# risingwavelabs/risingwave

Measured on AMD Instinct MI355X. Metric: input rows/sec/GPU on Nexmark q7 stream, higher is better.
Workload: dtype int64; 1 GPU; nexmark_q7; chunk_rows=4096, chunks_per_epoch_step=4096, windows_per_epoch=64, barriers=one checkpoint flush per step (a step = one epoch), agg=max(price), count group by 10s window (append-only), parallelism=dp1

## Files before the change

### include/rw_stream.h

```cpp
#ifndef RW_STREAM_H
#define RW_STREAM_H

#include "rw_chunk.h"

#ifdef __cplusplus
extern "C" {
#endif

#define RW_OK 0
#define RW_E_INVAL (-1)
#define RW_E_OVERFLOW (-2)
#define RW_E_INCONSISTENT (-3)
#define RW_E_NOGPU (-4)
#define RW_E_INTERNAL (-5)

const char* rw_last_error(void);
void rw_chunk_free(RwChunk* c);


enum RwAggKind {
    RW_AGG_COUNT_STAR = 0,
    RW_AGG_COUNT = 1,
    RW_AGG_SUM = 2,
    RW_AGG_SUM0 = 3,
// ... 94 lines not shown

void* rw_hash_join_create(const RwHashJoinDesc* desc);
int rw_hash_join_push_chunk(void* h, int side, const RwChunk* chunk);
int rw_hash_join_flush(void* h, uint64_t epoch);
int rw_hash_join_ingest_mode(void* h, int epoch_batched);
RwChunk* rw_hash_join_poll(void* h);
void rw_hash_join_destroy(void* h);

int rw_hash_join_watermark(void* h, int side, uint32_t col_idx, int64_t val,
                           uint32_t* out_cols, int64_t* out_vals, int max_out);

int rw_hash_agg_watermark(void* h, uint32_t group_key_pos, int64_t val);

int rw_hash_agg_update_vnode_bitmap(void* h, const uint8_t* bitmap,
                                    uint32_t vnode_count);
int rw_hash_join_update_vnode_bitmap(void* h, const uint8_t* bitmap,
                                     uint32_t vnode_count);

typedef struct RwGroupTopNDesc {
    uint32_t n_cols;
    const uint8_t* types;
    uint32_t n_group_by;
    const uint32_t* group_by;
    uint32_t n_order_by;
    const uint32_t* order_cols;
    const uint8_t* order_desc;
    uint32_t n_rest;
    const uint32_t* rest_cols;
    const uint8_t* rest_desc;
    uint64_t offset;
    uint64_t limit;
    uint8_t with_ties;
    uint32_t chunk_size;
    uint64_t state_capacity_hint;
    uint64_t row_capacity_hint;
} RwGroupTopNDesc;

void* rw_group_top_n_create(const RwGroupTopNDesc* desc);
int rw_group_top_n_push_chunk(void* h, const RwChunk* chunk);
int rw_group_top_n_flush(void* h, uint64_t epoch);
RwChunk* rw_group_top_n_poll(void* h);
void rw_group_top_n_destroy(void* h);

int rw_agg_checkpoint_drain(void* h, uint8_t** buf, uint64_t* len);
int rw_hash_agg_restore(void* h, const uint8_t* buf, uint64_t len);
int rw_agg_n_minput_tables(void* h);
int rw_agg_minput_drain(void* h, int mi, uint8_t** buf, uint64_t* len);
int rw_agg_minput_restore(void* h, int mi, const uint8_t* buf, uint64_t len);
int rw_hash_join_restore(void* h, int side, const uint8_t* buf, uint64_t len,
                         const uint8_t* deg_buf, uint64_t deg_len);
int rw_join_checkpoint_drain(void* h, int side, uint8_t** buf, uint64_t* len);
int rw_join_compact(void* h, int side, uint64_t* reclaimed);

int rw_hash_join_varlen_reserve(void* h, int side, uint64_t bytes);
int rw_hash_join_varlen_stats(void* h, int side, uint64_t* used,
                              uint64_t* capacity);
int rw_hash_join_varlen_emit_stats(void* h, double* ms, double* copy_ms,
                                   uint64_t* bytes, uint64_t* launches);
int rw_hash_agg_varlen_reserve(void* h, uint64_t arena_bytes,
                               uint64_t n_strings);
int rw_hash_agg_varlen_stats(void* h, uint64_t* arena_used,
                             uint64_t* arena_cap, uint64_t* n_strings,
                             uint64_t* table_cap);
int rw_hash_agg_varlen_intern_stats(void* h, double* kernel_ms,
                                    double* fetch_ms, uint64_t* launches);
int rw_agg_minput_compact(void* h, uint64_t* reclaimed);
int rw_topn_compact(void* h, uint64_t* reclaimed);
int rw_topn_checkpoint_drain(void* h, uint8_t** buf, uint64_t* len);
int rw_topn_restore(void* h, const uint8_t* buf, uint64_t len);
int rw_group_top_n_watermark(void* h, uint32_t col_idx, int64_t val);
int rw_agg_n_dedup_tables(void* h);
int rw_agg_dedup_drain(void* h, int di, uint8_t** buf, uint64_t* len);
int rw_agg_dedup_restore(void* h, int di, const uint8_t* buf, uint64_t len);
int rw_join_degree_drain(void* h, int side, uint8_t** buf, uint64_t* len);
void rw_spill_free(uint8_t* buf);

int rw_agg_apply_flush_launch(void* h, void* batch, uint32_t r0, uint32_t r1,
                              uint64_t epoch);
int rw_agg_debug_set_fuse(void* h, int mode);
int rw_agg_debug_fuse_allowed(void* h);
long long rw_agg_debug_fused_launches(void* h);
uint32_t rw_agg_debug_fuse_max(void);

#ifdef __cplusplus
}
#endif
#endif
```

### risingwave_amd/csrc/rw_amd.hip

```cpp

#include <hip/hip_runtime.h>

#include <cstdint>
#include <cstdio>
#include <cstdlib>
#include <cstring>
#include <map>
#include <new>
#include <optional>
#include <string>
#include <unordered_set>
#include <vector>

#include <rocprim/device/device_scan.hpp>

#include "../../include/rw_codec.hpp"
#include "../../include/rw_stream.h"
#include "../../include/rw_varlen.hpp"
#include "../../include/rw_xpayload.hpp"

#define WAVE 64

static thread_local std::string g_err;

// ... 5421 lines not shown
            }
        } else if (active && mhead != UINT32_MAX) {
            uint32_t row = mhead;
            while (row != UINT32_MAX) {
                JoinRowHdr* h = jrow(match, row);
                uint32_t vb = ld_u32(&h->validbits);
                if (ld_u32(&h->alive) &&
                    jhdr_key_eq(h, m.key_cols[1 - S], m.KW, kw, nullmask,
                                true) &&
                    join_cond_ok(m, S, b, r, vb, jvals(h))) {
                    const long long* mv = jvals(h);
                    jemit_row(out, m, S, op, b, r, vb,
                              [&](int col) {
                                  return ld_i64((const int64_t*)&mv[col]);
                              },
                              3);
                    matched_row = row;
                }
                row = ld_u32(&h->next);
            }
        }

        if (!m.append_only) {
            if (r < r1) {
                uint32_t myrow = *row_base + r;
                bool do_insert = active && is_insert;
                if (myrow < own.row_cap) {
                    JoinRowHdr* hd2 = jrow(own, myrow);
                    if (do_insert) {
                        long long* hv2 = jvals(hd2);
                        uint32_t vb2 = 0;
                        if (dense) {
                            for (int c = 0; c < m.n_cols[S]; c++)
                                hv2[c] = b.col_vals[c][r];
                            vb2 = (1u << m.n_cols[S]) - 1;
                            hd2->validbits = vb2;
                            hd2->degree = 0;
                            hd2->alive = 1;
                        } else if (b.all_insert) {
                            for (int c = 0; c < m.n_cols[S]; c++) {
                                hv2[c] = b.col_vals[c][r];
                                vb2 |= (uint32_t)(b.col_valid[c][r] != 0) << c;
                            }
                            hd2->validbits = vb2;
                            hd2->degree = 0;
                            hd2->alive = 1;
                        } else {
                            for (int c = 0; c < m.n_cols[S]; c++) {
                                st_i64((int64_t*)&hv2[c], b.col_vals[c][r]);
                                vb2 |= (uint32_t)(b.col_valid[c][r] != 0) << c;
                            }
                            st_u32(&hd2->validbits, vb2);
                            st_u32(&hd2->degree, 0);
                            st_u32(&hd2->alive, 1);
                        }
                        jbucket_insert(own, h64, myrow, !b.all_insert);
                    } else {
                        hd2->alive = 0;
                    }
                }
                if (active && !is_insert)
                    jown_delete(own, m, S, b, r, kw, nullmask);
            }
            continue;
        }
        if (!active) continue;

        if (m.append_only && is_insert && matched_row != UINT32_MAX) {
            st_u32(&jrow(match, matched_row)->alive, 0);
            if (match.killed) {
                uint32_t kidx = atomicAdd(match.killed_cursor, 1u);
                if (kidx < match.killed_cap) match.killed[kidx] = matched_row;
            }
            continue;
        }

        if (is_insert)
            jown_insert(own, m, S, b, r, kw, nullmask, out, 0);
        else
            jown_delete(own, m, S, b, r, kw, nullmask);
    }
}

__global__ void join_restore_kernel(JoinBatchDev b, JoinSideDev sd,
                                    JoinMeta m, int S,
                                    const uint32_t* degrees, uint32_t* err) {
    uint32_t stride = gridDim.x * blockDim.x;
    int lane = threadIdx.x & 63;
    uint32_t n = b.n_rows;
    uint32_t iters = (n + stride - 1) / stride;
    for (uint32_t it = 0; it < iters; it++) {
        uint32_t r = it * stride + blockIdx.x * blockDim.x + threadIdx.x;
        bool active = r < n;
        uint64_t wmask = __ballot(active);
        if (!active) continue;
        int leader = 63 - __clzll(wmask);
        uint32_t base = 0;
        if (lane == leader)
            base = atomicAdd(sd.row_cursor, (uint32_t)__popcll(wmask));
        base = (uint32_t)__shfl((int)base, leader);
        uint32_t row = base + (uint32_t)__popcll(wmask & ((1ULL << lane) - 1));
        if (row >= sd.row_cap) {
            atomicExch(err, 3u);
            continue;
        }
        JoinRowHdr* hd = jrow(sd, row);
        long long* hv = jvals(hd);
        uint32_t vb = 0;
        for (int c = 0; c < m.n_cols[S]; c++) {
            hv[c] = b.col_vals[c][r];
            vb |= (uint32_t)(b.col_valid[c][r] != 0) << c;
        }
        hd->validbits = vb;
        hd->degree = degrees ? degrees[r] : 0;
        hd->alive = 1;
        int64_t kw[MAX_KW];
        uint32_t nm = 0;
        for (int i = 0; i < m.KW; i++) {
            uint8_t col = m.key_cols[S][i];
            bool valid = (vb >> col) & 1;
            kw[i] = valid ? hv[col] : 0;
            nm |= (uint32_t)(!valid) << i;
        }
        jbucket_insert(sd, hash_key(kw, nm, m.KW), row, false);
    }
}

__global__ void jgather_rows_kernel(JoinSideDev sd, const uint32_t* ids,
                                    uint32_t n, uint8_t* out) {
    uint32_t stride = gridDim.x * blockDim.x;
    for (uint32_t i = blockIdx.x * blockDim.x + threadIdx.x; i < n;
         i += stride) {
        const uint8_t* src = sd.rows + (size_t)ids[i] * sd.row_stride;
        uint8_t* dst = out + (size_t)i * sd.row_stride;
        for (uint32_t w = 0; w < sd.row_stride; w += 8)
            *(long long*)(dst + w) = *(const long long*)(src + w);
    }
}

__global__ void jcompact_copy_kernel(JoinSideDev oldsd, uint8_t* nrows,
                                     uint32_t* ncursor, uint32_t old_n) {
    uint32_t stride = gridDim.x * blockDim.x;
    int lane = threadIdx.x & 63;
    uint32_t iters = (old_n + stride - 1) / stride;
    for (uint32_t it = 0; it < iters; it++) {
        uint32_t r = it * stride + blockIdx.x * blockDim.x + threadIdx.x;
        bool alive = r < old_n && jrow(oldsd, r)->alive;
        uint64_t wmask = __ballot(alive);
        if (!alive) continue;
        int leader = 63 - __clzll(wmask);
        uint32_t base = 0;
        if (lane == leader)
            base = atomicAdd(ncursor, (uint32_t)__popcll(wmask));
        base = (uint32_t)__shfl((int)base, leader);
        uint32_t nr = base + (uint32_t)__popcll(wmask & ((1ULL << lane) - 1));
        const uint8_t* src = oldsd.rows + (size_t)r * oldsd.row_stride;
        uint8_t* dst = nrows + (size_t)nr * oldsd.row_stride;
        for (uint32_t wq = 0; wq < oldsd.row_stride; wq += 8)
            *(long long*)(dst + wq) = *(const long long*)(src + wq);
        ((JoinRowHdr*)dst)->next = UINT32_MAX;
    }
}

__global__ void jcompact_link_kernel(JoinSideDev sd, JoinMeta m, int S,
                                     uint32_t n) {
    uint32_t stride = gridDim.x * blockDim.x;
// ... 609 lines not shown
    HIP_TRY(rocprim::exclusive_scan(d_scan_tmp, tmp, d_vlens, d_voffs,
                                    (uint64_t)0, (size_t)n + 1,
                                    rocprim::plus<uint64_t>(), stream));
    uint64_t total = 0;
    HIP_TRY(hipMemcpyAsync(&total, d_voffs + n, 8, hipMemcpyDeviceToHost,
                           stream));
    HIP_TRY(hipStreamSynchronize(stream));
    if (total) {
        uint64_t padded = total + VARLEN_COPY_PAD;
        if (d_vbytes_cap < padded) {
            if (d_vbytes) hipFree(d_vbytes);
            d_vbytes = nullptr;
            d_vbytes_cap = 0;
            uint64_t cap = 1ull << 16;
            while (cap < padded) cap <<= 1;
            HIP_TRY(hipMalloc(&d_vbytes, cap));
            d_vbytes_cap = cap;
        }
        if (timed) HIP_TRY(hipEventRecord(vev2, stream));
        varlen_copy_launch(v, arena, d_voffs, n, total, d_vbytes, stream);
    }
    if (timed) {
        HIP_TRY(hipEventRecord(vev1, stream));
        HIP_TRY(hipEventSynchronize(vev1));
        float ms = 0;
        HIP_TRY(hipEventElapsedTime(&ms, vev0, vev1));
        vemit_ms += ms;
        if (total) {
            HIP_TRY(hipEventElapsedTime(&ms, vev2, vev1));
            vcopy_ms += ms;
        }
        vemit_bytes += total;
        vemit_launches++;
    }
    HIP_TRY(hipMemcpy(offs.data(), d_voffs, ((size_t)n + 1) * 8,
                      hipMemcpyDeviceToHost));
    bytes.resize(total);
    if (total)
        HIP_TRY(hipMemcpy(bytes.data(), d_vbytes, total,
                          hipMemcpyDeviceToHost));
    return RW_OK;
}

VarlenFetch::~VarlenFetch() {
    if (d_vlens) hipFree(d_vlens);
    if (d_voffs) hipFree(d_voffs);
    if (d_vbytes) hipFree(d_vbytes);
    if (d_scan_tmp) hipFree(d_scan_tmp);
    if (vev0) {
        hipEventDestroy(vev0);
        hipEventDestroy(vev1);
        if (vev2) hipEventDestroy(vev2);
    }
}

struct HashJoin {
    RwHashJoinDesc desc;
    JoinMeta m{};
    JoinSideDev side[2]{};
    JoinOutDev out{};
    hipStream_t stream;
    std::vector<uint8_t> out_types;
    std::vector<uint8_t> types[2];
    JoinBatchDev stage[2]{};
    uint32_t stage_cap[2] = {0, 0};
    std::vector<RwChunk*> outq;
    uint8_t* zeros = nullptr;
    uint8_t* d_vnode_bitmap = nullptr;
    uint16_t* d_vnode_hop = nullptr;
    uint32_t d_vnode_hop_cap = 0;
    struct Wm { bool has = false; int64_t val = 0; };
    std::vector<uint32_t> wm_pos;
    std::vector<uint8_t> wm_clean;
    std::vector<Wm> wm_side0, wm_side1, wm_out;
    std::vector<uint32_t> ineq_col[2];
    std::vector<uint8_t> ineq_larger, ineq_do_clean;
    std::vector<Wm> ineq_wm[2], ineq_out;
    static constexpr int EV_RING = 256;
    hipEvent_t ev0[EV_RING] = {}, ev1[EV_RING] = {};
    uint8_t ev_pending[EV_RING] = {};
    uint64_t ev_head = 0;
    double probe_ms_total = 0;
    uint64_t probe_launches = 0, probe_rows = 0;

    int ev_harvest(int slot) {
        if (!ev_pending[slot]) return RW_OK;
        HIP_TRY(hipEventSynchronize(ev1[slot]));
        float ms = 0;
        HIP_TRY(hipEventElapsedTime(&ms, ev0[slot], ev1[slot]));
        probe_ms_total += ms;
        ev_pending[slot] = 0;
        return RW_OK;
    }
    int ev_harvest_all() {
        for (int s = 0; s < EV_RING; s++)
            if (ev_harvest(s) != RW_OK) return RW_E_INTERNAL;
        return RW_OK;
    }

    int init(const RwHashJoinDesc* d) {
        if (!gpu_ok()) FAIL(RW_E_NOGPU, "risingwave_amd: no GPU visible (product path has no CPU fallback)");
        desc = *d;
        if (d->join_type > RW_JOIN_RIGHT_ANTI)
            FAIL(RW_E_INVAL, "unknown join type %d", d->join_type);
        if (d->append_only && d->join_type != RW_JOIN_INNER)
            FAIL(RW_E_INVAL, "append-only optimize kernel is inner-only this round");
        if (d->n_key < 1 || d->n_key > MAX_KW) FAIL(RW_E_INVAL, "n_key %u", d->n_key);
        if (d->n_cols_l > MAX_COLS || d->n_cols_r > MAX_COLS)
            FAIL(RW_E_INVAL, "too many columns for round-1 kernels");
        if (d->n_output > MAX_OUT) FAIL(RW_E_INVAL, "too many output columns");
        m.KW = (int)d->n_key;
        m.n_cols[0] = (int)d->n_cols_l;
        m.n_cols[1] = (int)d->n_cols_r;
        m.n_pk[0] = (int)d->n_pk_l;
        m.n_pk[1] = (int)d->n_pk_r;
        types[0].assign(d->types_l, d->types_l + d->n_cols_l);
        types[1].assign(d->types_r, d->types_r + d->n_cols_r);
        for (int s = 0; s < 2; s++)
            for (size_t c = 0; c < types[s].size(); c++) {
                uint8_t t = types[s][c];
                if (t == RW_T_VARCHAR)
                    m.vc_mask[s] |= (uint8_t)(1u << c);
                else if (t != RW_T_I64 && t != RW_T_TS)
                    FAIL(RW_E_INVAL, "column type %d unsupported on GPU "
                                     "(i64/ts, varchar payload only)", t);
            }
        {
            const char* sn[2] = {"left", "right"};
            auto is_vc = [&](int s, uint32_t col) {
                return col < types[s].size() && types[s][col] == RW_T_VARCHAR;
            };
            auto is_vc_cat = [&](uint32_t idx) {
                return idx < d->n_cols_l ? is_vc(0, idx)
                                         : is_vc(1, idx - d->n_cols_l);
            };
            for (uint32_t i = 0; i < d->n_key; i++) {
                if (is_vc(0, d->key_l[i]))
                    FAIL(RW_E_INVAL, "varchar %s column %u cannot be a join key",
                         sn[0], d->key_l[i]);
                if (is_vc(1, d->key_r[i]))
                    FAIL(RW_E_INVAL, "varchar %s column %u cannot be a join key",
                         sn[1], d->key_r[i]);
            }
            for (uint32_t i = 0; i < d->n_pk_l; i++)
                if (is_vc(0, d->pk_l[i]))
                    FAIL(RW_E_INVAL, "varchar %s column %u cannot be a pk column",
                         sn[0], d->pk_l[i]);
            for (uint32_t i = 0; i < d->n_pk_r; i++)
                if (is_vc(1, d->pk_r[i]))
                    FAIL(RW_E_INVAL, "varchar %s column %u cannot be a pk column",
                         sn[1], d->pk_r[i]);
            if (d->has_cond && (is_vc_cat(d->cond_l) || is_vc_cat(d->cond_r)))
                FAIL(RW_E_INVAL, "varchar column %u cannot be a condition operand",
                     is_vc_cat(d->cond_l) ? d->cond_l : d->cond_r);
            if (d->has_cond && d->has_cond2 &&
                (is_vc_cat(d->cond2_l) || is_vc_cat(d->cond2_r)))
                FAIL(RW_E_INVAL, "varchar column %u cannot be a condition operand",
                     is_vc_cat(d->cond2_l) ? d->cond2_l : d->cond2_r);
            for (uint32_t p = 0; p < d->n_ineq; p++) {
                if (is_vc(0, d->ineq_left_col[p]))
                    FAIL(RW_E_INVAL, "varchar %s column %u cannot be an "
                                     "inequality/watermark column",
                         sn[0], d->ineq_left_col[p]);
                if (is_vc(1, d->ineq_right_col[p]))
                    FAIL(RW_E_INVAL, "varchar %s column %u cannot be an "
                                     "inequality/watermark column",
                         sn[1], d->ineq_right_col[p]);
            }
        }
        for (uint32_t i = 0; i < d->n_key; i++) {
            m.key_cols[0][i] = (uint8_t)d->key_l[i];
            m.key_cols[1][i] = (uint8_t)d->key_r[i];
            if (d->null_safe[i]) m.null_safe_mask |= 1 << i;
        }
        if (d->n_pk_l > MAX_KW || d->n_pk_r > MAX_KW) FAIL(RW_E_INVAL, "pk too wide");
        for (uint32_t i = 0; i < d->n_pk_l; i++) m.pk_cols[0][i] = (uint8_t)d->pk_l[i];
        for (uint32_t i = 0; i < d->n_pk_r; i++) m.pk_cols[1][i] = (uint8_t)d->pk_r[i];
        m.n_out = (int)d->n_output;
        for (uint32_t i = 0; i < d->n_output; i++) {
            uint32_t idx = d->output_indices[i];
            if (idx < d->n_cols_l) {
                m.out_src[i] = 0;
                m.out_col[i] = (uint8_t)idx;
                out_types.push_back(types[0][idx]);
            } else {
                m.out_src[i] = 1;
                m.out_col[i] = (uint8_t)(idx - d->n_cols_l);
                out_types.push_back(types[1][idx - d->n_cols_l]);
            }
        }
        auto split = [&](uint32_t idx, uint8_t* src, uint8_t* col) {
            if (idx < d->n_cols_l) {
                *src = 0;
                *col = (uint8_t)idx;
            } else {
                *src = 1;
                *col = (uint8_t)(idx - d->n_cols_l);
            }
        };
        m.n_cond = 0;
        if (d->has_cond) {
            m.cond[0].op = d->cond_op;
            split(d->cond_l, &m.cond[0].src_l, &m.cond[0].col_l);
            split(d->cond_r, &m.cond[0].src_r, &m.cond[0].col_r);
            m.cond[0].rconst = d->cond_rconst;
            m.n_cond = 1;
            if (d->has_cond2) {
                m.cond[1].op = d->cond2_op;
                split(d->cond2_l, &m.cond[1].src_l, &m.cond[1].col_l);
                split(d->cond2_r, &m.cond[1].src_r, &m.cond[1].col_r);
                m.cond[1].rconst = d->cond2_rconst;
                m.n_cond = 2;
            }
        }
        m.append_only = d->append_only;
        m.join_type = d->join_type;
        m.need_deg[0] = j_need_degree(d->join_type, RW_SIDE_LEFT);
        m.need_deg[1] = j_need_degree(d->join_type, RW_SIDE_RIGHT);
        if (d->n_wm_jk) {
            wm_pos.assign(d->wm_jk_pos, d->wm_jk_pos + d->n_wm_jk);
            wm_clean.assign(d->wm_jk_clean, d->wm_jk_clean + d->n_wm_jk);
        }
        wm_side0.resize(d->n_key);
        wm_side1.resize(d->n_key);
        wm_out.resize(d->n_key);
        if (d->n_ineq) {
            ineq_col[0].assign(d->ineq_left_col,
                               d->ineq_left_col + d->n_ineq);
            ineq_col[1].assign(d->ineq_right_col,
                               d->ineq_right_col + d->n_ineq);
            ineq_larger.assign(d->ineq_left_larger,
                               d->ineq_left_larger + d->n_ineq);
            ineq_do_clean.assign(d->ineq_clean, d->ineq_clean + d->n_ineq);
            ineq_wm[0].resize(d->n_ineq);
            ineq_wm[1].resize(d->n_ineq);
            ineq_out.resize(d->n_ineq);
        }

        HIP_TRY(hipStreamCreate(&stream));
        uint64_t key_cap = d->state_capacity_hint ? d->state_capacity_hint : (1u << 20);
        uint64_t row_cap = d->row_capacity_hint ? d->row_capacity_hint : (1u << 22);
        for (int s = 0; s < 2; s++) {
            uint32_t cap = 1;
            while (cap < key_cap * 2) cap <<= 1;
            JoinSideDev& js = side[s];
            js.cap_mask = cap - 1;
            js.slots = nullptr;
            HIP_TRY(hipMalloc(&js.slots8, (size_t)cap * 8));
            HIP_TRY(hipMemsetAsync(js.slots8, 0, (size_t)cap * 8, stream));
            js.row_cap = (uint32_t)row_cap;
            uint32_t rs = 16 + 8 * (uint32_t)m.n_cols[s];
            if (rs > 32 && rs <= 64) rs = 64;
            else if (rs > 64) rs = (rs + 31) & ~31u;
            js.row_stride = rs;
            HIP_TRY(hipMalloc(&js.rows, (size_t)row_cap * js.row_stride));
            HIP_TRY(hipMalloc(&js.row_cursor, 4));
            HIP_TRY(hipMemset(js.row_cursor, 0, 4));
            js.killed_cap = 1u << 22;
            HIP_TRY(hipMalloc(&js.killed, (size_t)js.killed_cap * 4));
            HIP_TRY(hipMalloc(&js.killed_cursor, 4));
            HIP_TRY(hipMemset(js.killed_cursor, 0, 4));
            js.deg_dirty_flag = nullptr;
            js.deg_dirty_list = nullptr;
            js.deg_dirty_n = nullptr;
            if (m.need_deg[s]) {
                HIP_TRY(hipMalloc(&js.deg_dirty_flag, (size_t)row_cap * 4));
                HIP_TRY(hipMemset(js.deg_dirty_flag, 0, (size_t)row_cap * 4));
                HIP_TRY(hipMalloc(&js.deg_dirty_list, (size_t)row_cap * 4));
                HIP_TRY(hipMalloc(&js.deg_dirty_n, 4));
                HIP_TRY(hipMemset(js.deg_dirty_n, 0, 4));
            }
        }
        HIP_TRY(hipStreamSynchronize(stream));
        out.cap = 1u << 22;
        HIP_TRY(hipMalloc(&out.vals, (size_t)out.cap * m.n_out * 8));
        HIP_TRY(hipMalloc(&out.nulls, (size_t)out.cap * m.n_out));
        HIP_TRY(hipMalloc(&out.ops, out.cap));
        HIP_TRY(hipMalloc(&out.counters, 8));
        HIP_TRY(hipMemset(out.counters, 0, 8));
        return RW_OK;
    }

    int ensure_stage(int s, uint32_t n) {
        if (stage_cap[s] >= n) return RW_OK;
        for (int c = 0; c < m.n_cols[s]; c++) {
            if (stage[s].col_vals[c]) hipFree(stage[s].col_vals[c]);
            if (stage[s].col_valid[c]) hipFree(stage[s].col_valid[c]);
        }
        if (stage[s].ops) hipFree(stage[s].ops);
        if (stage[s].vis) hipFree(stage[s].vis);
        uint32_t cap = 4096;
        while (cap < n) cap <<= 1;
        for (int c = 0; c < m.n_cols[s]; c++) {
            HIP_TRY(hipMalloc(&stage[s].col_vals[c], (size_t)cap * 8));
            HIP_TRY(hipMalloc(&stage[s].col_valid[c], cap));
        }
        HIP_TRY(hipMalloc(&stage[s].ops, cap));
        HIP_TRY(hipMalloc(&stage[s].vis, cap));
        stage_cap[s] = cap;
        return RW_OK;
    }

    static constexpr uint64_t ARENA_DEFAULT = 1ull << 20;
    uint64_t arena_used[2] = {0, 0};
    uint64_t arena_cap[2] = {0, 0};
    uint64_t arena_reserve[2] = {0, 0};
    bool seen_input = false;
    std::vector<int64_t> vwords[2][MAX_COLS];
    VarlenFetch vf;

    bool has_varchar() const { return (m.vc_mask[0] | m.vc_mask[1]) != 0; }

    int arena_ensure(int s, uint64_t extra) {
        uint64_t need = arena_used[s] + extra;
        if (need > rwvarlen::MAX_OFF)
            FAIL(RW_E_INVAL, "varchar arena would exceed 2^40-1 bytes");
        if (side[s].arena && need <= arena_cap[s]) return RW_OK;
        uint64_t cap = arena_cap[s] ? arena_cap[s]
                       : arena_reserve[s] ? arena_reserve[s] : ARENA_DEFAULT;
        while (cap < need) cap *= 2;
        uint8_t* na = nullptr;
// ... 12 lines not shown

    int ensure_vscratch(uint32_t n) { return vf.ensure_vscratch(n); }
    int varlen_fetch(const VarlenView& v, const uint8_t* arena, uint32_t n,
                     std::vector<uint64_t>& offs, std::vector<uint8_t>& bytes,
                     bool timed) {
        return vf.fetch(v, arena, n, offs, bytes, timed, stream);
    }

    int upload(int s, const RwChunk* c, JoinBatchDev* bout) {
        uint32_t n = c->n_rows;
        for (int ci = 0; m.vc_mask[s] && ci < m.n_cols[s]; ci++) {
            if (!((m.vc_mask[s] >> ci) & 1)) continue;
            if (c->cols[ci].type != RW_T_VARCHAR)
                FAIL(RW_E_INVAL, "column %d: expected a varchar column", ci);
            auto* vd = (const RwVarlenData*)c->cols[ci].data;
            const char* why =
                vd ? rwvarlen::validate_offsets(vd->offsets, n) : "data is NULL";
            if (why) FAIL(RW_E_INVAL, "varchar column %d: %s", ci, why);
            if (n && vd->offsets[n] && !vd->bytes)
                FAIL(RW_E_INVAL, "varchar column %d: bytes is NULL", ci);
        }
        seen_input = true;
        int rc = ensure_stage(s, n);
        if (rc != RW_OK) return rc;
        JoinBatchDev b = stage[s];
        for (int ci = 0; ci < m.n_cols[s]; ci++) {
            if ((m.vc_mask[s] >> ci) & 1) {
                auto* vd = (const RwVarlenData*)c->cols[ci].data;
                uint64_t total = n ? vd->offsets[n] : 0;
                rc = arena_ensure(s, total);
                if (rc != RW_OK) return rc;
                uint64_t base = arena_used[s];
                if (total)
                    HIP_TRY(hipMemcpyAsync(side[s].arena + base, vd->bytes,
                                           total, hipMemcpyHostToDevice,
                                           stream));
                arena_used[s] += total;
                auto& w = vwords[s][ci];
                w.resize(n);
                for (uint32_t r = 0; r < n; r++)
                    w[r] = c->cols[ci].valid[r]
                               ? (int64_t)rwvarlen::pack(
                                     base + vd->offsets[r],
                                     vd->offsets[r + 1] - vd->offsets[r])
                               : 0;
                HIP_TRY(hipMemcpyAsync(b.col_vals[ci], w.data(), (size_t)n * 8,
                                       hipMemcpyHostToDevice, stream));
                HIP_TRY(hipMemcpyAsync(b.col_valid[ci], c->cols[ci].valid, n,
                                       hipMemcpyHostToDevice, stream));
                continue;
            }
            HIP_TRY(hipMemcpyAsync(b.col_vals[ci], c->cols[ci].data, (size_t)n * 8,
                                   hipMemcpyHostToDevice, stream));
            HIP_TRY(hipMemcpyAsync(b.col_valid[ci], c->cols[ci].valid, n,
                                   hipMemcpyHostToDevice, stream));
        }
        HIP_TRY(hipMemcpyAsync(b.ops, c->ops, n, hipMemcpyHostToDevice, stream));
        if (c->vis)
            HIP_TRY(hipMemcpyAsync(b.vis, c->vis, n, hipMemcpyHostToDevice, stream));
        else
            b.vis = nullptr;
        b.n_rows = n;
        b.all_insert = 1;
        for (uint32_t r = 0; r < n && b.all_insert; r++)
            if (!(c->vis && !c->vis[r]) && c->ops[r] != RW_OP_INSERT &&
                c->ops[r] != RW_OP_UPDATE_INSERT)
                b.all_insert = 0;
        b.all_valid = 1;
        for (int ci = 0; ci < m.n_cols[s] && b.all_valid; ci++)
            for (uint32_t r = 0; r < n && b.all_valid; r++)
                b.all_valid = c->cols[ci].valid[r];
        b.unique_keys = 0;
        *bout = b;
        return RW_OK;
    }

    uint32_t* d_probe_base = nullptr;
    unsigned long long* d_emit_count = nullptr;
    uint8_t* d_vis_scratch = nullptr;
    uint32_t d_vis_cap = 0;
    uint32_t last_sparse_rows = 0;
    bool sparse_out = false;

    int probe(int s, const JoinBatchDev& b, bool timed, uint32_t r0, uint32_t r1) {
        uint32_t blocks = (r1 - r0 + 255) / 256;
        if (blocks > 16384) blocks = 16384;
        if (!blocks) blocks = 1;
        int slot = -1;
        if (timed) {
            slot = (int)(ev_head++ % EV_RING);
            if (!ev0[slot]) {
                HIP_TRY(hipEventCreate(&ev0[slot]));
                HIP_TRY(hipEventCreate(&ev1[slot]));
            }
            if (ev_harvest(slot) != RW_OK) return RW_E_INTERNAL;
            HIP_TRY(hipEventRecord(ev0[slot], stream));
        }
        if (m.join_type == RW_JOIN_INNER && !m.append_only && r0 == 0) {
            if (!d_probe_base) {
                HIP_TRY(hipMalloc(&d_probe_base, 4));
                HIP_TRY(hipMalloc(&d_emit_count, 8));
            }
            if (b.n_rows > out.cap)
                FAIL(RW_E_INVAL, "probe batch larger than the output block");
            HIP_TRY(hipMemsetAsync(out.ops, 0xFF, b.n_rows, stream));
            jprobe_setup_kernel<<<1, 1, 0, stream>>>(
                out, side[s].row_cursor, side[s].row_cap, d_probe_base,
                b.n_rows);
            last_sparse_rows = b.n_rows;
            sparse_out = true;
        }
        if (m.join_type != RW_JOIN_INNER) {
            join_probe_noninner_kernel<<<blocks, 256, 0, stream>>>(
                b, side[s], side[1 - s], m, s, out, r0, r1);
        } else {
            join_probe_kernel<<<blocks, 256, 0, stream>>>(
                b, side[s], side[1 - s], m, s, out, r0, r1, d_probe_base);
        }
        if (timed) {
            HIP_TRY(hipEventRecord(ev1[slot], stream));
            ev_pending[slot] = 1;
            probe_launches++;
            probe_rows += b.n_rows;
        }
        return RW_OK;
    }

    uint32_t flush_mark[2] = {0, 0};
    uint8_t* compact_scratch[2] = {nullptr, nullptr};
    int checkpoint_drain(int s, std::vector<uint8_t>& sp) {
        HIP_TRY(hipStreamSynchronize(stream));
        JoinSideDev& js = side[s];
        uint32_t cur = 0, kcur = 0;
        HIP_TRY(hipMemcpy(&cur, js.row_cursor, 4, hipMemcpyDeviceToHost));
        HIP_TRY(hipMemcpy(&kcur, js.killed_cursor, 4, hipMemcpyDeviceToHost));
        if (kcur > js.killed_cap)
            FAIL(RW_E_INTERNAL, "join kill list overflow (lost deltas)");
        if (cur > js.row_cap) cur = js.row_cap;
        uint32_t mark = flush_mark[s];
        size_t stride = js.row_stride;
        std::vector<uint8_t> fresh((size_t)(cur - mark) * stride);
        if (cur > mark)
            HIP_TRY(hipMemcpy(fresh.data(), js.rows + (size_t)mark * stride,
                              fresh.size(), hipMemcpyDeviceToHost));
        std::vector<uint32_t> kills(kcur);
        if (kcur)
            HIP_TRY(hipMemcpy(kills.data(), js.killed, (size_t)kcur * 4,
                              hipMemcpyDeviceToHost));
        auto encode_key = [&](const uint8_t* rec, std::string& k) {
            const uint32_t vb = ((const uint32_t*)rec)[2];
            const int64_t* vals = (const int64_t*)(rec + 16);
            std::vector<uint8_t> kb;
            auto put_datum = [&](uint8_t col) {
                rwcodec::DatumC d{!((vb >> col) & 1), vals[col], 0};
                rwcodec::memcmp_encode_datum(kb, types[s][col], d, {});
            };
            for (int i = 0; i < m.KW; i++) put_datum(m.key_cols[s][i]);
            for (int i = 0; i < m.n_pk[s]; i++) put_datum(m.pk_cols[s][i]);
            k.assign((const char*)kb.data(), kb.size());
        };
        std::vector<std::vector<uint64_t>> voffs(m.n_cols[s]);
        std::vector<std::vector<uint8_t>> vbytes(m.n_cols[s]);
        if (m.vc_mask[s] && cur > mark) {
            uint32_t nf = cur - mark;
            std::vector<uint64_t> words(nf);
            uint64_t* d_words = nullptr;
            HIP_TRY(hipMalloc(&d_words, (size_t)nf * 8));
            for (int c = 0; c < m.n_cols[s]; c++) {
                if (!((m.vc_mask[s] >> c) & 1)) continue;
                for (uint32_t i = 0; i < nf; i++) {
                    const uint8_t* rec = fresh.data() + (size_t)i * stride;
                    const uint32_t* hd = (const uint32_t*)rec;
                    bool live = hd[0] && ((hd[2] >> c) & 1);
                    words[i] = live ? ((const uint64_t*)(rec + 16))[c] : 0;
                }
                if (hipMemcpy(d_words, words.data(), (size_t)nf * 8,
                              hipMemcpyHostToDevice) != hipSuccess) {
                    hipFree(d_words);
                    FAIL(RW_E_INTERNAL, "drain string gather failed");
                }
                VarlenView v{};
                v.words = d_words;
                v.stride = 1;
                int rcv = varlen_fetch(v, js.arena, nf, voffs[c], vbytes[c],
                                       false);
                if (rcv != RW_OK) {
                    hipFree(d_words);
                    return rcv;
                }
            }
            hipFree(d_words);
        }
        auto encode_val = [&](const uint8_t* rec, std::vector<uint8_t>& v) {
            const uint32_t vb = ((const uint32_t*)rec)[2];
            const int64_t* vals = (const int64_t*)(rec + 16);
            for (int c = 0; c < m.n_cols[s]; c++) {
                if ((m.vc_mask[s] >> c) & 1) {
// ... 1264 lines not shown
            VarlenView v{};
            v.words = (const uint64_t*)(sd.rows + 16) + c;
            v.stride = sd.row_stride / 8;
            uint32_t blocks = (n_alive + 1 + 255) / 256;
            if (blocks > 4096) blocks = 4096;
            varlen_len_kernel<<<blocks, 256, 0, j->stream>>>(v, n_alive,
                                                             j->vf.d_vlens);
            size_t tmp = 0;
            if (rocprim::exclusive_scan(nullptr, tmp, j->vf.d_vlens, j->vf.d_voffs,
                                        (uint64_t)0, (size_t)n_alive + 1,
                                        rocprim::plus<uint64_t>(),
                                        j->stream) != hipSuccess) {
                rcv = RW_E_INTERNAL;
                break;
            }
            if (tmp > j->vf.d_scan_tmp_cap) {
                if (j->vf.d_scan_tmp) hipFree(j->vf.d_scan_tmp);
                j->vf.d_scan_tmp = nullptr;
                j->vf.d_scan_tmp_cap = 0;
                if (hipMalloc(&j->vf.d_scan_tmp, tmp) != hipSuccess) {
                    rcv = RW_E_INTERNAL;
                    break;
                }
                j->vf.d_scan_tmp_cap = tmp;
            }
            uint64_t total = 0;
            if (rocprim::exclusive_scan(j->vf.d_scan_tmp, tmp, j->vf.d_vlens,
                                        j->vf.d_voffs, (uint64_t)0,
                                        (size_t)n_alive + 1,
                                        rocprim::plus<uint64_t>(),
                                        j->stream) != hipSuccess ||
                hipMemcpyAsync(&total, j->vf.d_voffs + n_alive, 8,
                               hipMemcpyDeviceToHost, j->stream) != hipSuccess ||
                hipStreamSynchronize(j->stream) != hipSuccess) {
                rcv = RW_E_INTERNAL;
                break;
            }
            uint64_t base = (new_used + VARLEN_COPY_PAD - 1) &
                            ~(uint64_t)(VARLEN_COPY_PAD - 1);
            if (total)
                varlen_copy_launch(v, sd.arena, j->vf.d_voffs, n_alive, total,
                                   na + base, j->stream);
            uint32_t rblocks = (n_alive + 255) / 256;
            if (rblocks > 4096) rblocks = 4096;
            varlen_rewrite_kernel<<<rblocks, 256, 0, j->stream>>>(
                sd, c, n_alive, j->vf.d_voffs, base);
            if (hipStreamSynchronize(j->stream) != hipSuccess) {
                rcv = RW_E_INTERNAL;
                break;
            }
            new_used = base + total;
        }
        if (rcv != RW_OK) {
            hipFree(na);
            FAIL(RW_E_INTERNAL, "compact: arena rebuild failed");
        }
        hipFree(sd.arena);
        sd.arena = na;
        if (j->arena_used[side] > new_used)
            arena_freed = j->arena_used[side] - new_used;
        j->arena_used[side] = new_used;
    }
    if (reclaimed)
        *reclaimed = (uint64_t)(cur - n_alive) * sd.row_stride + arena_freed;
    return RW_OK;
}

int rw_join_degree_drain(void* h, int side, uint8_t** buf, uint64_t* len) {
    auto* j = (HashJoin*)h;
    if (side != 0 && side != 1) FAIL(RW_E_INVAL, "bad side");
    auto& sp = j->deg_spill[side];
    int rc = spill_export(sp, buf, len);
    if (rc != RW_OK) return rc;
    sp.clear();
    return RW_OK;
}

int rw_join_stats_reset(void* h) {
    auto* j = (HashJoin*)h;
    j->ev_harvest_all();
    j->probe_launches = 0;
    j->probe_ms_total = 0;
    j->probe_rows = 0;
    return RW_OK;
}

}


#define TOPN_MAX_CK 8
#define TOPN_MAX_WIN 128

struct TopMeta {
    int KW;
    int n_cols;
    uint8_t gk_cols[MAX_KW];
    uint8_t gk_float[MAX_KW];
    int n_ck;
    uint8_t ck_cols[TOPN_MAX_CK];
    uint8_t ck_desc[TOPN_MAX_CK];
    uint8_t ck_float[TOPN_MAX_CK];
    uint32_t offset, limit;
    uint8_t with_ties;
    int n_order;
};

__device__ __forceinline__ int topn_cmp(const TopMeta& m, const long long* va,
                                        uint32_t nba, const long long* vb,
                                        uint32_t nbb, int ncols) {
    for (int i = 0; i < ncols; i++) {
        int c = m.ck_cols[i];
        bool na = !((nba >> c) & 1), nb = !((nbb >> c) & 1);
        int r;
        if (na || nb) {
            r = (na && nb) ? 0 : (na ? 1 : -1);
        } else if (m.ck_float[i]) {
            double da = __longlong_as_double(va[c]);
            double db = __longlong_as_double(vb[c]);
            bool an = isnan(da), bn = isnan(db);
            if (an || bn) r = an == bn ? 0 : (an ? 1 : -1);
            else r = da < db ? -1 : (da > db ? 1 : 0);
        } else {
            r = va[c] < vb[c] ? -1 : (va[c] > vb[c] ? 1 : 0);
        }
        if (m.ck_desc[i]) r = -r;
        if (r) return r;
    }
    return 0;
}

__device__ __forceinline__ bool topn_ck_eq_batch(const TopMeta& m,
                                                 const JoinBatchDev& b,
                                                 uint32_t r, const long long* v,
                                                 uint32_t nb) {
    for (int i = 0; i < m.n_ck; i++) {
        int c = m.ck_cols[i];
        bool bn = !b.col_valid[c][r];
        bool rn = !((nb >> c) & 1);
        if (bn != rn) return false;
        if (!bn && b.col_vals[c][r] != v[c]) return false;
    }
    return true;
}

__device__ __forceinline__ int64_t fkey_canon(int64_t w) {
    double d = __longlong_as_double((long long)w);
    if (d == 0.0) return 0;
    if (d != d) return 0x7ff8000000000000LL;
    return w;
}

__device__ __forceinline__ int64_t topn_gkw(const TopMeta& m, int i,
                                            int64_t v) {
    return m.gk_float[i] ? fkey_canon(v) : v;
}

__global__ void topn_touch_kernel(JoinBatchDev b, JoinSideDev sd, TopMeta m,
                                  uint32_t* touched, uint32_t* touched_list,
                                  uint32_t* counters ) {
    uint32_t stride = gridDim.x * blockDim.x;
    for (uint32_t r = blockIdx.x * blockDim.x + threadIdx.x; r < b.n_rows;
         r += stride) {
        if (b.vis && !b.vis[r]) continue;
        int64_t kw[MAX_KW];
        uint32_t nullmask = 0;
        for (int i = 0; i < m.KW; i++) {
// ... 1075 lines not shown
```

Measured before the change: 305.4 billion rows/s.

## Add register-resident dense inner-join probe kernel and sample probe timing events

Adds a specialized inner-join probe kernel for the case where all rows are valid inserts and rows are narrow. It loads probe values and matched rows into registers with vector loads and writes every output op directly, so the output memset can be skipped. It also records probe timing events only on a sampled subset of launches to cut event overhead, and makes the block cap configurable. The new kernel adds a specialized path and duplicates the insert/match logic, which risks divergence from the generic kernel.

```diff
diff --git a/include/rw_stream.h b/include/rw_stream.h
--- a/include/rw_stream.h
+++ b/include/rw_stream.h
@@ -200,6 +200,9 @@
 long long rw_agg_debug_fused_launches(void* h);
 uint32_t rw_agg_debug_fuse_max(void);
 
+long long rw_join_debug_fast_launches(void* h);
+int rw_join_debug_set_max_blocks(void* h, uint32_t n);
+
 #ifdef __cplusplus
 }
 #endif
diff --git a/risingwave_amd/csrc/rw_amd.hip b/risingwave_amd/csrc/rw_amd.hip
--- a/risingwave_amd/csrc/rw_amd.hip
+++ b/risingwave_amd/csrc/rw_amd.hip
@@ -5527,6 +5527,195 @@
     }
 }
 
+__device__ __forceinline__ bool join_cond_ok_regs(const JoinMeta& m,
+                                                  int probe_side,
+                                                  const long long* pv,
+                                                  uint32_t validbits,
+                                                  const long long* recv) {
+    bool ok = true;
+#pragma unroll
+    for (int ci = 0; ci < 2; ci++) {
+        if (ci < m.n_cond) {
+            auto& cd = m.cond[ci];
+            bool lp = (int)cd.src_l == probe_side;
+            bool rp = (int)cd.src_r == probe_side;
+            if (!lp && !((validbits >> cd.col_l) & 1)) ok = false;
+            if (!rp && !((validbits >> cd.col_r) & 1)) ok = false;
+            long long a = lp ? rec_sel(pv, cd.col_l) : rec_sel(recv, cd.col_l);
+            long long c = rp ? rec_sel(pv, cd.col_r) : rec_sel(recv, cd.col_r);
+            c += cd.rconst;
+            bool t;
+            switch (cd.op) {
+                case RW_CMP_LT: t = a < c; break;
+                case RW_CMP_LE: t = a <= c; break;
+                case RW_CMP_GT: t = a > c; break;
+                case RW_CMP_GE: t = a >= c; break;
+                default: t = false;
+            }
+            ok = ok && t;
+        }
+    }
+    return ok;
+}
+
+template <typename MVal>
+__device__ __forceinline__ void jwrite_row_regs(JoinOutDev& out, int n_out,
+                                                uint64_t out_sel,
+                                                const long long* pv,
+                                                uint32_t match_vb, MVal mval,
+                                                uint32_t orow) {
+    jout_store<true>(&out.ops[orow], (uint8_t)RW_OP_INSERT);
+    int64_t* vp = out.vals + orow;
+    uint8_t* np = out.nulls + orow;
+#pragma nounroll
+    for (int c = 0; c < n_out; c++) {
+        int col = (int)(out_sel & 7);
+        bool from_probe = !(out_sel & 8);
+        out_sel >>= 4;
+        uint8_t valid = from_probe ? 1 : (uint8_t)((match_vb >> col) & 1);
+        int64_t v = from_probe ? rec_sel(pv, col) : mval(col);
+        jout_store<true>(vp, valid ? v : (int64_t)0);
+        jout_store<true>(np, (uint8_t)!valid);
+        vp += out.cap;
+        np += out.cap;
+    }
+}
+
+struct JoinDenseDesc {
+    uint64_t out_sel[2];
+};
+
+__global__ __launch_bounds__(256, 6) void join_probe_dense_kernel(
+    JoinBatchDev b, JoinSideDev own, JoinSideDev match, JoinMeta m, int S,
+    JoinOutDev out, uint32_t r0, uint32_t r1, const uint32_t* row_base,
+    JoinDenseDesc dd) {
+    uint32_t stride = gridDim.x * blockDim.x;
+    uint32_t n = r1 - r0;
+    uint32_t iters = (n + stride - 1) / stride;
+    const int ncp = m.n_cols[S];
+    const uint64_t out_sel = dd.out_sel[S];
+    const int nw16 = (int)(match.row_stride >> 4);
+    const uint32_t rbase = *row_base;
+
+    for (uint32_t it = 0; it < iters; it++) {
+        uint32_t r = r0 + it * stride + blockIdx.x * blockDim.x + threadIdx.x;
+        if (r >= r1) continue;
+        long long pv[6];
+#pragma unroll
+        for (int c = 0; c < 6; c++) pv[c] = c < ncp ? b.col_vals[c][r] : 0;
+        uint64_t h64 = 0x20210401u;
+        long long kw[MAX_KW];
+#pragma unroll
+        for (int i = 0; i < MAX_KW; i++) {
+            kw[i] = 0;
+            if (i < m.KW) {
+                kw[i] = rec_sel(pv, m.key_cols[S][i]);
+                h64 = mix64(h64 ^ (uint64_t)kw[i]);
+            }
+        }
+        uint64_t* oslot = &own.slots8[jslot_start(h64, own.cap_mask)];
+        const uint64_t* mslot =
+            &match.slots8[jslot_start(h64, match.cap_mask)];
+        uint64_t old = __hip_atomic_load(oslot, RLX);
+        uint64_t mpacked = *mslot;
+        __builtin_amdgcn_sched_barrier(0);
+        uint32_t mhead = ((uint32_t)mpacked & jbloom_bit(h64))
+                             ? jhead_of(mpacked)
+                             : UINT32_MAX;
+
+        long long rec[8];
+        auto load_rec = [&](uint32_t row) {
+            const long long* rp = (const long long*)jrow(match, row);
+#pragma unroll
+            for (int w = 0; w < 4; w++)
+                if (w < nw16)
+                    *(longlong2*)&rec[2 * w] = *(const longlong2*)(rp + 2 * w);
+        };
+        auto rec_ok = [&]() {
+            uint32_t vb = (uint32_t)(uint64_t)rec[1];
+            bool eq = (uint32_t)(uint64_t)rec[0] != 0;
+#pragma unroll
+            for (int i = 0; i < MAX_KW; i++) {
+                if (i < m.KW) {
+                    int col = m.key_cols[1 - S][i];
+                    if (!((vb >> col) & 1) || rec_sel(rec + 2, col) != kw[i])
+                        eq = false;
+                }
+            }
+            return eq && join_cond_ok_regs(m, S, pv, vb, rec + 2);
+        };
+
+        uint32_t myrow = rbase + r;
+        bool have_row = myrow < own.row_cap;
+        auto want = [&](uint64_t o) {
+            return have_row ? ((uint64_t)myrow << 32) |
+                                  ((uint32_t)o | jbloom_bit(h64))
+                            : o;
+        };
+        uint64_t prev = atomicCAS((unsigned long long*)oslot, old, want(old));
+        uint32_t row = mhead;
+
+        uint32_t my_n = 0;
+        bool rec_match = false;
+        while (row != UINT32_MAX) {
+            load_rec(row);
+            rec_match = rec_ok();
+            if (rec_match) my_n++;
+            row = (uint32_t)((uint64_t)rec[0] >> 32);
+        }
+        asm volatile("" : "+v"(prev));
+        while (prev != old) {
+            old = prev;
+            prev = atomicCAS((unsigned long long*)oslot, old, want(old));
+        }
+
+        if (have_row) {
+            uint32_t next = (uint32_t)old ? jhead_of(old) : UINT32_MAX;
+            longlong2* dst = (longlong2*)jrow(own, myrow);
+            longlong2 hdr;
+            hdr.x = (long long)(((uint64_t)next << 32) | 1u);
+            hdr.y = (long long)(uint64_t)((1u << ncp) - 1);
+            dst[0] = hdr;
+#pragma unroll
+            for (int w = 0; w < 3; w++)
+                if (2 * w < ncp) {
+                    longlong2 cell;
+                    cell.x = pv[2 * w];
+                    cell.y = pv[2 * w + 1];
+                    dst[1 + w] = cell;
+                }
+        }
+        uint32_t extra_base = 0;
+        bool overflow = false;
+        if (my_n > 1) {
+            extra_base = atomicAdd(&out.counters[0], my_n - 1);
+            overflow = extra_base + my_n - 1 > out.cap;
+            if (overflow) atomicExch(&out.counters[1], 1u);
+        }
+        if (my_n == 1 && rec_match) {
+            jwrite_row_regs(
+                out, m.n_out, out_sel, pv, (uint32_t)(uint64_t)rec[1],
+                [&](int col) { return rec_sel(rec + 2, col); }, r);
+        } else if (my_n && !overflow) {
+            uint32_t k = 0;
+            row = mhead;
+            while (row != UINT32_MAX && k < my_n) {
+                load_rec(row);
+                if (rec_ok()) {
+                    jwrite_row_regs(
+                        out, m.n_out, out_sel, pv, (uint32_t)(uint64_t)rec[1],
+                        [&](int col) { return rec_sel(rec + 2, col); },
+                        k == 0 ? r : extra_base + k - 1);
+                    k++;
+                }
+                row = (uint32_t)((uint64_t)rec[0] >> 32);
+            }
+        } else {
+            jout_store<true>(&out.ops[r], (uint8_t)0xFF);
+        }
+    }
+}
+
 __global__ void join_restore_kernel(JoinBatchDev b, JoinSideDev sd,
                                     JoinMeta m, int S,
                                     const uint32_t* degrees, uint32_t* err) {
@@ -6302,6 +6491,12 @@
     uint64_t ev_head = 0;
     double probe_ms_total = 0;
     uint64_t probe_launches = 0, probe_rows = 0;
+    uint32_t ev_every = 16;
+    uint64_t ev_tick = 0;
+    bool fast_enabled = true;
+    uint64_t fast_launches = 0;
+    uint32_t max_blocks = 16384;
+    JoinDenseDesc dense_desc{};
 
     int ev_harvest(int slot) {
         if (!ev_pending[slot]) return RW_OK;
@@ -6409,6 +6604,11 @@
                 out_types.push_back(types[1][idx - d->n_cols_l]);
             }
         }
+        for (int ps = 0; ps < 2; ps++)
+            for (int i = 0; i < m.n_out; i++)
+                dense_desc.out_sel[ps] |=
+                    (uint64_t)((m.out_col[i] & 7) | (m.out_src[i] == ps ? 0 : 8))
+                    << (4 * i);
         auto split = [&](uint32_t idx, uint8_t* src, uint8_t* col) {
             if (idx < d->n_cols_l) {
                 *src = 0;
@@ -6457,6 +6657,11 @@
             ineq_out.resize(d->n_ineq);
         }
 
+        if (const char* e = getenv("RW_JOIN_FAST")) fast_enabled = atoi(e) != 0;
+        if (const char* e = getenv("RW_JOIN_EVENT_EVERY")) {
+            int v = atoi(e);
+            if (v >= 1) ev_every = (uint32_t)v;
+        }
         HIP_TRY(hipStreamCreate(&stream));
         uint64_t key_cap = d->state_capacity_hint ? d->state_capacity_hint : (1u << 20);
         uint64_t row_cap = d->row_capacity_hint ? d->row_capacity_hint : (1u << 22);
@@ -6635,11 +6840,25 @@
     uint32_t last_sparse_rows = 0;
     bool sparse_out = false;
 
+    bool dense_fast(int s, const JoinBatchDev& b) const {
+        auto narrow = [](const JoinSideDev& js) {
+            return js.row_stride <= 64 && !(js.row_stride & 15);
+        };
+        return fast_enabled && m.join_type == RW_JOIN_INNER &&
+               !m.append_only && b.all_insert && b.all_valid && !b.vis &&
+               narrow(side[0]) && narrow(side[1]) && !m.vc_mask[0] &&
+               !m.vc_mask[1];
+    }
+
     int probe(int s, const JoinBatchDev& b, bool timed, uint32_t r0, uint32_t r1) {
         uint32_t blocks = (r1 - r0 + 255) / 256;
-        if (blocks > 16384) blocks = 16384;
+        if (blocks > max_blocks) blocks = max_blocks;
         if (!blocks) blocks = 1;
         int slot = -1;
+        if (timed) {
+            uint64_t t = ev_tick++;
+            if (t % ev_every != (t / ev_every) % ev_every) timed = false;
+        }
         if (timed) {
             slot = (int)(ev_head++ % EV_RING);
             if (!ev0[slot]) {
@@ -6649,6 +6868,7 @@
             if (ev_harvest(slot) != RW_OK) return RW_E_INTERNAL;
             HIP_TRY(hipEventRecord(ev0[slot], stream));
         }
+        const bool fast = dense_fast(s, b);
         if (m.join_type == RW_JOIN_INNER && !m.append_only && r0 == 0) {
             if (!d_probe_base) {
                 HIP_TRY(hipMalloc(&d_probe_base, 4));
@@ -6656,7 +6876,8 @@
             }
             if (b.n_rows > out.cap)
                 FAIL(RW_E_INVAL, "probe batch larger than the output block");
-            HIP_TRY(hipMemsetAsync(out.ops, 0xFF, b.n_rows, stream));
+            if (!fast)
+                HIP_TRY(hipMemsetAsync(out.ops, 0xFF, b.n_rows, stream));
             jprobe_setup_kernel<<<1, 1, 0, stream>>>(
                 out, side[s].row_cursor, side[s].row_cap, d_probe_base,
                 b.n_rows);
@@ -6666,6 +6887,11 @@
         if (m.join_type != RW_JOIN_INNER) {
             join_probe_noninner_kernel<<<blocks, 256, 0, stream>>>(
                 b, side[s], side[1 - s], m, s, out, r0, r1);
+        } else if (fast) {
+            join_probe_dense_kernel<<<blocks, 256, 0, stream>>>(
+                b, side[s], side[1 - s], m, s, out, r0, r1, d_probe_base,
+                dense_desc);
+            fast_launches++;
         } else {
             join_probe_kernel<<<blocks, 256, 0, stream>>>(
                 b, side[s], side[1 - s], m, s, out, r0, r1, d_probe_base);
@@ -8096,6 +8322,17 @@
     j->probe_launches = 0;
     j->probe_ms_total = 0;
     j->probe_rows = 0;
+    j->ev_tick = 0;
+    return RW_OK;
+}
+
+long long rw_join_debug_fast_launches(void* h) {
+    return (long long)((HashJoin*)h)->fast_launches;
+}
+
+int rw_join_debug_set_max_blocks(void* h, uint32_t n) {
+    if (n < 1 || n > 16384) FAIL(RW_E_INVAL, "max_blocks %u", n);
+    ((HashJoin*)h)->max_blocks = n;
     return RW_OK;
 }
 
```

New measurement: 284.8 billion rows/s. 0.933x the previous value.
